# honglianghe/CDNet

Hardware: AMD Instinct MI355X
Metric: tiles/sec (train fwd+bwd+Adam), 256x256 (higher is better)
Workload: dtype fp32

## Files before the change

cdnet_amd/_lib.py:

```python
import ctypes as C
import os

_HERE = os.path.dirname(os.path.abspath(__file__))
LIB_PATH = os.environ.get('CDNET_LIB_PATH') or os.path.join(_HERE, 'libcdnet_hip.so')

_vp, _i, _sz, _f, _u = C.c_void_p, C.c_int, C.c_size_t, C.c_float, C.c_uint

class WgradReduceDesc(C.Structure):
    _fields_ = [('slab', C.c_void_p), ('dw', C.c_void_p)] + [(n, C.c_int) for n in (
        'ksplit', 'npar', 'ci_blocks', 'co_blocks', 'taps', 'CI', 'CO', 'Csrc_real', 'Cin_real', 'src_coff', 'Cout', 'mode', 'block0', 'blocks')]


SIGNATURES = {
    'cdnet_abi_version': (_i, []),
    'cdnet_abi_sizeof': (_sz, [C.c_char_p]),
    'cdnet_last_error': (C.c_char_p, []),
    'cdnet_build_info': (C.c_char_p, []),
    'cdnet_spin': (_i, [_i, _vp]),
    'cdnet_box_copy': (_i, [_vp, _vp, _sz, _vp]),
    'cdnet_box_mfma': (_i, [_vp, _vp, _vp, _i, _i, _i, _vp]),
    'cdnet_ddm_codes': (_i, [_vp, _i, _i, _i, _i, _vp, _i, _i, _vp, _vp, _vp]),
    'cdnet_ddm_normalize': (_i, [_vp, _vp, _i, _i, _i, _vp, _vp]),
    'cdnet_probmaps': (_i, [_vp, _vp, _i, _i, _i, _i, _vp, _vp, _vp]),
    'cdnet_tta_boost_argmax': (_i, [_vp, _vp, _vp, _vp, _i, _i, _vp, _i, _i, _vp, _vp, _vp, _vp, _vp, _vp]),
    'cdnet_fuse_sum': (_i, [_vp, _i, _i, _i, _i, _i, _i, _vp, _i, _i, _vp]),
    'cdnet_upsample_bilinear_backward': (_i, [_vp, _i, _i, _i, _i, _i, _i, _i, _i, _vp, _vp]),
    'cdnet_s2d_to_nhwc': (_i, [_vp, _i, _i, _i, _i, _vp, _vp]),
    'cdnet_fuse_sum_f32': (_i, [_vp, _i, _i, _i, _i, _i, _i, _vp, _i, _i, _vp]),
    'cdnet_upsample_bilinear_backward_f32': (_i, [_vp, _i, _i, _i, _i, _i, _i, _i, _i, _vp, _vp]),
    'cdnet_s2d_to_nhwc_f32': (_i, [_vp, _i, _i, _i, _i, _vp, _vp]),
    'cdnet_bn_backward_stats': (_i, [_vp, _vp, _vp, _vp, _vp, _sz, _vp, _vp]),
    'cdnet_bn_backward_apply': (_i, [_vp, _vp, _vp, _vp]),
    'cdnet_bn_backward_finalize': (_i, [_vp, _vp, _vp, _vp, _vp, _i, _vp, _vp]),
    'cdnet_conv_ws_eligible': (_i, [_vp]),
    'cdnet_grad_sum': (_i, [_vp, _i, _vp, C.c_longlong, _i, _vp, _vp]),
    'cdnet_grad_sum_f32': (_i, [_vp, _i, _vp, C.c_longlong, _i, _vp, _vp]),
    'cdnet_label_pair_histogram': (_i, [_vp, _vp, _i, _i, _i, _i, _vp, _vp, _vp, _vp, _vp, _vp]),
    'cdnet_remap_label': (_i, [_vp, _i, _i, _i, _vp, _vp, _vp, _vp]),
    'cdnet_label_areas': (_i, [_vp, _i, _i, _i, _vp, _vp, _vp]),
    'cdnet_label_apply': (_i, [_vp, _i, _i, _i, _vp, _vp, _vp]),
    'cdnet_label_csr_workspace_bytes': (_sz, [_i]),
    'cdnet_label_csr': (_i, [_vp, _i, _i, _i, _vp, _sz, _vp, _vp, _vp, _vp, _vp]),
    'cdnet_hausdorff_tile_pixels': (_i, []),
    'cdnet_hausdorff_chunk_pixels': (_i, []),
    'cdnet_hausdorff_pairs': (_i, [_vp] * 8 + [_i, _i, _i, _vp, _i, _vp, _i, _vp, _vp, _vp]),
    'cdnet_watershed_workspace_bytes': (_sz, [_i, _i, _i]),
    'cdnet_watershed_process': (_i, [_vp, _i, _i, _i, _i, _vp, _sz, _vp, _vp, _vp, _vp]),
    'cdnet_fill_label_process': (_i, [_vp, _i, _i, _i, _i, _vp, _sz, _vp, _vp]),
    'cdnet_tile_postproc_workspace_bytes': (_sz, [_i, _i, _i, _i]),
    'cdnet_tile_postproc': (_i, [_vp, _vp, _vp, _i, _i, _i, _i, _vp, _i, _i, _i, _i, _vp, _sz] + [_vp] * 10),
    'cdnet_cc_workspace_bytes': (_sz, [_i, _i, _i]),
    'cdnet_cc_chain': (_i, [_vp, _i, _i, _i, _i, _i, _i, _vp, _sz, _vp, _vp, _vp, _vp, _vp, _vp]),
    'cdnet_mask_views_argmax': (_i, [_vp, _i, _i, _i, _vp, _i, _i, _vp, _vp, _vp]),
    'cdnet_tile_mask_postproc_workspace_bytes': (_sz, [_i, _i, _i, _i]),
    'cdnet_tile_mask_postproc': (_i, [_vp, _i, _i, _i, _i, _i, _i, _vp, _sz] + [_vp] * 8),
    'cdnet_dilate_labels': (_i, [_vp, _i, _i, _i, _i, _vp, _vp]),
    'cdnet_conv_packed_weight_elems': (_sz, [_i] * 6),
# ... 122 lines not shown
```

cdnet_amd/csrc/build.py:

```python
import os
import subprocess
import sys

HERE = os.path.dirname(os.path.abspath(__file__))
PKG = os.path.dirname(HERE)
LIB = os.path.join(PKG, 'libcdnet_hip.so')
OBJ_DIR = os.path.join(HERE, 'build')
SOURCES = ['abi.hip', 'box.hip', 'postproc.hip', 'postproc_tile.hip', 'conv.hip', 'conv32.hip', 'conv32ws.hip', 'conv16ws.hip', 'wgrad.hip', 'model.hip', 'head_bwd.hip', 'dam_loss.hip', 'bn_bwd.hip', 'cdm.hip', 'metrics.hip', 'augment.hip', 'optim.hip', 'variance.hip', 'boundary.hip', 'mask_loss.hip']
FLAGS = ['--offload-arch=gfx950', '-O3', '-std=c++20', '-fPIC', '-ffp-contract=off', '-Wall',
         '-Wno-unused-function', '-Wno-unused-result']


def _newer(a, bs):
    return os.path.exists(a) and all(os.path.getmtime(a) >= os.path.getmtime(b) for b in bs)


def build(force=False, verbose=False):
    hipcc = os.environ.get('HIPCC', 'hipcc')
    flags = FLAGS + os.environ.get('CDNET_HIPCC_FLAGS', '').split()
    os.makedirs(OBJ_DIR, exist_ok=True)
    headers = [os.path.join(HERE, f) for f in os.listdir(HERE) if f.endswith('.h')]
    headers.append(os.path.join(os.path.dirname(PKG), 'include', 'cdnet_hip.h'))
    objs, procs = [], []
    for s in SOURCES:
        src = os.path.join(HERE, s)
        if not os.path.exists(src):
            continue
        obj = os.path.join(OBJ_DIR, s.replace('.hip', '.o'))
        objs.append(obj)
        if force or not _newer(obj, [src] + headers):
            cmd = [hipcc] + flags + ['-c', src, '-o', obj]
# ... 17 lines not shown
```

cdnet_amd/csrc/conv32.hip:

```cpp
#include <type_traits>
#include "common.h"
#include "conv_args.h"
#include "launch.h"
#include <stdlib.h>

using namespace cdnet;

typedef __attribute__((ext_vector_type(8))) __bf16 bf16x8;
typedef __attribute__((ext_vector_type(2))) __bf16 bf16x2;
typedef __attribute__((ext_vector_type(16))) float f32x16;
typedef __attribute__((ext_vector_type(2))) float f32x2;
typedef unsigned u32x4 __attribute__((ext_vector_type(4)));
typedef float f32x4 __attribute__((ext_vector_type(4)));

namespace {

__device__ __forceinline__ void split8(const float *v, u32x4 &hi, u32x4 &lo) {
#pragma unroll
    for (int k = 0; k < 4; ++k) {
        const f32x2 x = {v[2 * k], v[2 * k + 1]};
        const bf16x2 h = __builtin_convertvector(x, bf16x2);
        const unsigned hb = __builtin_bit_cast(unsigned, h);
        const f32x2 hf = {__builtin_bit_cast(float, hb << 16), __builtin_bit_cast(float, hb & 0xffff0000u)};
        const bf16x2 l = __builtin_convertvector(x - hf, bf16x2);
// ... 610 lines not shown
                }
#pragma unroll
                for (int q = 0; q < 4; ++q) {
                    const float4 t = xf(raw[q], nullptr);
                    if (q == 0) val = t;
                    else if (ok[q]) { val.x = fmaxf(val.x, t.x); val.y = fmaxf(val.y, t.y); val.z = fmaxf(val.z, t.z); val.w = fmaxf(val.w, t.w); }
                }
            }
        }
        *reinterpret_cast<float4 *>(out + pix * s.C + c) = val;
    }
}

}

namespace cdnet {

int conv_forward_f32(const ConvArgs &A, hipStream_t st) {
    CDNET_REQUIRE(A.CK == 16, "cdnet_conv_forward(f32): CK must be 16 (got %d)", A.CK);
    for (int i = 0; i < A.nsrc; ++i)
        CDNET_REQUIRE(!A.src[i].pool, "cdnet_conv_forward(f32): pooled sources must be materialised (cdnet_src_materialize)");
    CDNET_REQUIRE(!A.out_f16, "cdnet_conv_forward(f32): out_f16 must be 0");
    {
        const int rc = conv_forward_f32_ws(A, st);
        if (rc >= 0) return rc;
    }
    CDNET_REQUIRE(A.ws != 2, "cdnet_conv_forward(f32): the BatchNorm-backward statistics epilogue (ws = 2) needs the producer / consumer kernel "
                             "(ask cdnet_conv_ws_eligible first)");
    CDNET_REQUIRE(A.taps1 == 0 || A.taps1 == A.taps, "cdnet_conv_forward(f32): a one-tap second source runs on conv_ws32_kernel only (ask cdnet_conv_ws_eligible)");
    CDNET_REQUIRE(!A.pool_out, "cdnet_conv_forward(f32): the fused max-pool output rides in conv_ws32_kernel's epilogue only (ask cdnet_conv_ws_eligible)");
    if (A.taps == 9) return dispatch_conv32<9>(A, st);
    if (A.taps == 4) return dispatch_conv32<4>(A, st);
    {
        const int rc = try_conv1x1_stream(A, st);
        if (rc >= 0) return rc;
    }
    return dispatch_conv32<1>(A, st);
}

int materialize_f32(const ConvSrc &s, int N, int H, int W, void *out, hipStream_t st) {
    const size_t total = (size_t)N * H * W * (s.C / 4);
    size_t g = (total + 255) / 256;
    g = g > 8192 ? 8192 : g;
    materialize_f32_kernel<<<(int)g, 256, 0, st>>>(s, N, H, W, reinterpret_cast<float *>(out));
    return check_launch("cdnet_src_materialize(f32)");
}

// ... 2 lines not shown
```

cdnet_amd/csrc/conv_args.h:

```cpp
#pragma once
#include "../../include/cdnet_hip.h"

struct ConvSrc {
    const unsigned short *x;
    const unsigned short *res;
    const float *scale;
    const float *shift;
    int C, Hs, Ws, pool, relu, off_y, off_x;
    int f16, row_stride;
};

struct ConvArgs {
    ConvSrc src[2];
    int nsrc;
    const unsigned short *w;
    const float *bias;
    const float *oscale;
    const float *oshift;
    int orelu;
    unsigned short *out;
    int Cout, out_cstride, out_coff;
    float *stats;
    int N, H, W;
    int taps, npar, ostride, nchunk;
    int tile, CK, BN;
    int out_f16;
    int debug;
    int ws;
    int f32;
    const unsigned short *eres;
    const float *eres_scale, *eres_shift;
    int eres_f16, eres_relu;
    int taps1, pad_;
    unsigned short *pool_out;
    const float *dot_w, *dot_b;
    float *dot_out;
};

enum : int {
    CONV_DBG_WS16_QUAD = 16,
    CONV_DBG_ONE_TILE = 32,
    CONV_DBG_PERSIST_SMALL = 64,
    CONV_DBG_OLD_WS16 = 128,
    CONV_DBG_NO_STREAM_1X1 = 256,
    CONV_DBG_GRID_SHIFT = 8,
};
enum : int {
    WGRAD_DBG_NO_WS = 8,
    WGRAD_DBG_ALL_QUADS = 16,
};

static_assert(sizeof(ConvSrc) == sizeof(cdnet_conv_src), "ConvSrc layout");
static_assert(sizeof(ConvArgs) == sizeof(cdnet_conv_args), "ConvArgs layout");

namespace cdnet {
int conv_forward_f32(const ConvArgs &A, hipStream_t st);
int conv_forward_f32_ws(const ConvArgs &A, hipStream_t st, bool dry_run = false);
int conv_forward_ws16(const ConvArgs &A, hipStream_t st, bool dry_run = false);
int materialize_f32(const ConvSrc &s, int N, int H, int W, void *out, hipStream_t st);
}
```

cdnet_amd/engine.py:

```python
import ctypes as C
import os
import torch

from . import _lib


class ConvSrc(C.Structure):
    _fields_ = [('x', C.c_void_p), ('res', C.c_void_p), ('scale', C.c_void_p), ('shift', C.c_void_p),
                ('C', C.c_int), ('Hs', C.c_int), ('Ws', C.c_int), ('pool', C.c_int), ('relu', C.c_int),
                ('off_y', C.c_int), ('off_x', C.c_int), ('f16', C.c_int), ('row_stride', C.c_int)]


class ConvArgs(C.Structure):
    _fields_ = [('src', ConvSrc * 2), ('nsrc', C.c_int), ('w', C.c_void_p), ('bias', C.c_void_p),
                ('oscale', C.c_void_p), ('oshift', C.c_void_p), ('orelu', C.c_int), ('out', C.c_void_p),
                ('Cout', C.c_int), ('out_cstride', C.c_int), ('out_coff', C.c_int), ('stats', C.c_void_p),
                ('N', C.c_int), ('H', C.c_int), ('W', C.c_int), ('taps', C.c_int), ('npar', C.c_int),
                ('ostride', C.c_int), ('nchunk', C.c_int), ('tile', C.c_int), ('CK', C.c_int), ('BN', C.c_int),
                ('out_f16', C.c_int), ('debug', C.c_int), ('ws', C.c_int), ('f32', C.c_int),
                ('eres', C.c_void_p), ('eres_scale', C.c_void_p), ('eres_shift', C.c_void_p), ('eres_f16', C.c_int), ('eres_relu', C.c_int),
                ('taps1', C.c_int), ('pad_', C.c_int), ('pool_out', C.c_void_p),
                ('dot_w', C.c_void_p), ('dot_b', C.c_void_p), ('dot_out', C.c_void_p)]


def _dp(t):
    return None if t is None else t.data_ptr()


class Src:

    def __init__(self, x, scale=None, shift=None, relu=False, pool=False, res=None, off=(0, 0), view=None):
        assert x.dtype in (torch.bfloat16, torch.float16, torch.float32) and x.is_contiguous()
        assert res is None or res.dtype == x.dtype
        self.x, self.scale, self.shift, self.relu, self.pool, self.res, self.off = x, scale, shift, relu, pool, res, off
        if view is None:
            assert x.dim() == 4
            self.N, self.Hs, self.Ws, self.Cc = x.shape
            self.ptr_off, self.row_stride = 0, 0
        else:
            self.ptr_off, self.Hs, self.Ws, self.Cc, self.row_stride = view
            self.N = x.shape[0]

    @property
    def f16(self):
# ... 125 lines not shown
            wp = torch.zeros((Cout, Cin_p, KH, KW), dtype=torch.float32, device=w.device)
            wp[:, :Cin] = w
        else:
            raise NotImplementedError
        w, Cin = wp.contiguous(), Cin_p
    n = packed_elems(Cout, Cin // CK, taps, CK, BN, npar) * (2 if split else 1)
    if out is None or out.numel() != n:
        out = torch.empty((n,), dtype=torch.int16, device=w.device)
    if cout_scale is not None:
        assert mode == 0 and cout_scale.dtype == torch.float32 and cout_scale.numel() == Cout
        _lib.call('cdnet_pack_conv_weights_scaled', _lib.ptr(w), _lib.ptr(cout_scale), _lib.ptr(out), Cout, Cin, KH, KW, CK, BN,
                  mode | (PACK_SPLIT if split else 0), _lib.stream_ptr())
        return out
    _lib.call('cdnet_pack_conv_weights', _lib.ptr(w), _lib.ptr(out), Cout, Cin, KH, KW, CK, BN, mode | (PACK_SPLIT if split else 0),
              _lib.stream_ptr())
    return out


CONV_DEBUG = 0


def conv_forward(srcs, wpacked, Cout, cfg, taps=9, transposed=False, bias=None, oscale=None, oshift=None,
                 orelu=False, out=None, stats=None, H=None, W=None, out_dtype=torch.bfloat16, eres=None, query_ws=False, bns=None, taps1=0, pool_out=None, dot=None,
                 pad_chunks=0, debug_or=0):
    tile, CK, BN = cfg[:3]
    s0 = srcs[0]
    f32 = s0.f32
    assert all(s.f32 == f32 for s in srcs)
    if f32:
        out_dtype = torch.float32
    N = s0.N
    if H is None:
        H, W = s0.logical_hw()
        H, W = H + 0, W + 0
    ostride = 2 if transposed else 1
    npar = 4 if transposed else 1
    a = ConvArgs()
    nchunk = 0
    for i, s in enumerate(srcs):
        assert s.C % CK == 0, (s.C, CK)
        s.fill(a.src[i])
        nchunk += s.C // CK
    a.nsrc = len(srcs)
    if dot is not None:
        assert out is None and stats is None and eres is None and bns is None and pool_out is None and not f32 and not transposed
        a.dot_w, a.dot_b, a.dot_out = dot[0].data_ptr(), dot[1].data_ptr(), dot[2].data_ptr()
        assert dot[0].numel() == Cout and dot[0].dtype == torch.float32 and dot[2].dtype == torch.float32 and dot[2].numel() == N * H * W
    elif out is None:
        out = torch.empty((N, H * ostride, W * ostride, Cout), dtype=out_dtype, device=s0.x.device)
    ntiles = ((H + tile - 1) // tile) * ((W + tile - 1) // tile)
    if stats is True:
        stats = torch.empty((N * npar * ntiles, 2, Cout), dtype=torch.float32, device=s0.x.device)
    a.w, a.bias, a.oscale, a.oshift = _dp(wpacked), _dp(bias), _dp(oscale), _dp(oshift)
    a.orelu = int(orelu)
    a.out, a.Cout, a.out_cstride, a.out_coff = (None if out is None else out.data_ptr()), Cout, (Cout if out is None else out.shape[3]), 0
    a.stats = _dp(stats)
    a.N, a.H, a.W = N, H, W
    assert pad_chunks == 0 or (len(srcs) == 2 and taps == 9 and not f32 and all(s.scale is None and not s.relu and s.res is None and not s.f16 for s in srcs))
    a.taps, a.npar, a.ostride, a.nchunk = taps, npar, ostride, nchunk + pad_chunks
    a.tile, a.CK, a.BN = tile, CK, BN
    a.out_f16 = int(out is not None and out.dtype == torch.float16)
    a.ws = 0
    a.taps1 = taps1
    a.pool_out = _dp(pool_out)
    a.debug = CONV_DEBUG | debug_or
    a.f32 = int(f32)
    assert out is None or (out.dtype == torch.float32) == f32
    if eres is not None:
        assert not transposed and stats is None and not orelu and out.dtype == (torch.float32 if f32 else torch.bfloat16) and tuple(eres.x.shape) == tuple(out.shape)
        assert eres.f32 == f32
        a.eres, a.eres_scale, a.eres_shift = eres.x.data_ptr(), _dp(eres.scale), _dp(eres.shift)
        a.eres_f16, a.eres_relu = int(eres.f16), int(eres.relu)
    if bns is not None:
        raw, sc, sh, mu, inv, partial = bns
        assert eres is None and stats is None and bias is None and oscale is None and oshift is None and tuple(raw.shape) == tuple(out.shape)
        a.ws = 2
        a.eres, a.oscale, a.oshift, a.eres_scale, a.eres_shift, a.stats = raw.data_ptr(), sc.data_ptr(), sh.data_ptr(), mu.data_ptr(), inv.data_ptr(), partial.data_ptr()
    if query_ws:
        return int(_lib.load().cdnet_conv_ws_eligible(C.byref(a)))
    _lib.call('cdnet_conv_forward', C.byref(a), _lib.stream_ptr())
    return out, stats
```

cdnet_amd/trainer.py:

```python
import ctypes as C
import os

import torch

from . import _lib, engine, optim, runtime, streams
from .allreduce import BucketReducer, bucketed_allreduce
from .engine import Src
from .optim import HEAD_PARAMS, FlatState
from .synth import synthetic_batch


class GradIn(C.Structure):
    _fields_ = [('g', C.c_void_p), ('Hg', C.c_int), ('Wg', C.c_int), ('oy', C.c_int), ('ox', C.c_int),
                ('pooled', C.c_int), ('coff', C.c_int), ('cstride', C.c_int), ('pad_', C.c_int)]


class BnBwdArgs(C.Structure):
    _fields_ = [('raw', C.c_void_p), ('res', C.c_void_p), ('scale', C.c_void_p), ('shift', C.c_void_p),
                ('mean', C.c_void_p), ('invstd', C.c_void_p), ('gin', GradIn * 3), ('ngin', C.c_int),
                ('f16', C.c_int), ('relu', C.c_int), ('N', C.c_int), ('H', C.c_int), ('W', C.c_int), ('C', C.c_int)]


_WGRAD_WGS_DEEP, _WGRAD_WGS_SHALLOW = 128, 160
_WGRAD_WGS_KQ = 128
# ... 575 lines not shown
        wpb, cfgb = L.backward_pack(cin_total, H, W)
        if L.kind == 'conv3s2':
            Cp = cin_total // 4
            gs2d = self.buf(('ds2d', L.name), (N, H, W, cin_total), runtime.act_dtype())
            engine.conv_forward([Src(g)], wpb, cin_total, cfgb, taps=9, out=gs2d, H=H, W=W)
            gin = self.buf(('din', L.name), (N, 2 * H, 2 * W, Cp), runtime.act_dtype())
            _lib.call(_lib.entry('cdnet_s2d_to_nhwc', gin.dtype == torch.float32), _lib.ptr(gs2d), N, H, W, Cp, _lib.ptr(gin),
                      _lib.stream_ptr())
            add(srcs[0].x, _G(gin, 2 * H, 2 * W))
            return
        if not L.transposed:
            gin = self.buf(('din', L.name), (N, H, W, cin_total), runtime.act_dtype())
            fuse = None if isinstance(g, Src) else self._stats_fusable(L, srcs, H, W, N, wpb, cfgb, cin_total)
            if fuse is not None:
                P, part = fuse
                engine.conv_forward([Src(g)], wpb, cin_total, cfgb, taps=L.taps, out=gin, H=H, W=W,
                                    bns=(srcs[0].x, P.scale, P.shift, P.save_mean, P.save_invstd, part))
                self._bn_partials[id(srcs[0].x)] = part
            else:
                engine.conv_forward([g if isinstance(g, Src) else Src(g)], wpb, cin_total, cfgb, taps=L.taps, out=gin, H=H, W=W)
        else:
            gin = self.buf(('din', L.name), (N, H, W, cin_total), runtime.act_dtype())
            views = [Src(g, view=(a * 2 * W * Cout, H, W, 2 * Cout, 4 * W * Cout)) for a in (0, 1)]
            engine.conv_forward(views, wpb, cin_total, cfgb, taps=(9 if L.kind == 'convT4' else 1), out=gin, H=H, W=W)
        coff = 0
        for s in srcs:
            if getattr(s, 'is_input', False):
                coff += s.C
                continue
            tgt, pool = getattr(s, 'grad_to', (s.x, int(s.pool)))
            add(tgt, _G(gin, H, W, oy=s.off[0], ox=s.off[1], pooled=pool, coff=coff, cstride=cin_total))
            coff += s.C

    def _overlap_begin(self):
        self._ar = None
        if not self._reduce_active() or os.environ.get('CDNET_ALLREDUCE_OVERLAP', '1') == '0':
            return
        f = self.flat
        base = f.G.data_ptr()
        pend = {}
        owners = [p for L in self.tape if not isinstance(L, runtime.FuseNode) for p in (L.weight, L.bias, None if L.bn is None else L.bn.weight,
                                                 None if L.bn is None else L.bn.bias) if p is not None]
        for p in owners:
            off = (p.grad.data_ptr() - base) // 4
            if 0 <= off < f.n_used:
                pend[off] = off + p.numel()
        if f.n_head:
# ... 204 lines not shown
```

include/cdnet_hip.h:

```cpp
#ifndef CDNET_HIP_H
#define CDNET_HIP_H

#include <stddef.h>
#include <stdint.h>

#ifdef __cplusplus
extern "C" {
#endif

#define CDNET_OK            0
#define CDNET_E_ARG         1
#define CDNET_E_WORKSPACE   2
#define CDNET_E_LAUNCH      3

#define CDNET_ABI_VERSION   5

int         cdnet_abi_version(void);
size_t      cdnet_abi_sizeof(const char *struct_name);
const char *cdnet_last_error(void);
const char *cdnet_build_info(void);
int         cdnet_spin(int microseconds, void *stream);
int         cdnet_box_copy(const void *src, void *dst, size_t bytes, void *stream);
int         cdnet_box_mfma(const uint32_t *seed, float *sink, unsigned long long *stamps, int workgroups, int waves_per_wg, int iters, void *stream);

// ... 56 lines not shown
    int nsrc;
    const uint16_t *w;
    const float *bias;
    const float *oscale;
    const float *oshift;
    int orelu;
    uint16_t *out;
    int Cout, out_cstride, out_coff;
    float *stats;
    int N, H, W;
    int taps;
    int npar;
    int ostride;
    int nchunk;
    int tile, CK, BN;
    int out_f16;
    int debug;
    int ws;
    int f32;
    const uint16_t *eres;
    const float *eres_scale, *eres_shift;
    int eres_f16, eres_relu;
    int taps1;
    int pad_;
    uint16_t *pool_out;
    const float *dot_w;
    const float *dot_b;
    float *dot_out;
} cdnet_conv_args;

size_t cdnet_conv_packed_weight_elems(int Cout, int nchunk, int taps, int CK, int BN, int npar);
#define CDNET_PACK_SPLIT 16
int cdnet_pack_conv_weights(const float *w, void *packed, int Cout, int Cin, int KH, int KW, int CK, int BN, int mode,
                            void *stream);
int cdnet_pack_conv_weights_scaled(const float *w, const float *cout_scale, void *packed, int Cout, int Cin, int KH, int KW, int CK,
                                   int BN, int mode, void *stream);
typedef struct cdnet_pack_job {
    const float *w;
    void *packed;
    int Cout, Cin, KH, KW, CK, BN, mode, pad_;
} cdnet_pack_job;
size_t cdnet_pack_batch_table_bytes(int n_jobs);
int cdnet_pack_conv_weights_batch(const cdnet_pack_job *jobs, int n_jobs, void *table, size_t table_bytes, int upload,
                                  void *stream);
int cdnet_conv_forward(const cdnet_conv_args *args, void *stream);

int cdnet_input_pack(const float *x, int N, int C, int H, int W, void *out_bf16_nhwc16, void *stream);
// ... 8 lines not shown
typedef struct cdnet_head_feat {
    const uint16_t *raw;
    const uint16_t *res;
    const float *scale;
    const float *shift;
    int relu;
    int f16;
} cdnet_head_feat;

#define CDNET_HEAD_WEIGHT_FLOATS 855
int cdnet_dam_head_forward(const cdnet_head_feat *f1, const cdnet_head_feat *f2, const cdnet_head_feat *f3,
                           const float *head_weights, int N, int H, int W, float *mask, float *point,
                           float *direction, void *stream);
int cdnet_final_conv1x1(const cdnet_head_feat *f, const float *w, const float *b, int K, int N, int H, int W,
                        float *out, void *stream);
size_t cdnet_bias_grad_workspace_floats(int C);
int cdnet_bias_grad(const uint16_t *grad_out, size_t npix, int C, float *workspace, size_t workspace_floats, float *db, void *stream);
int cdnet_bias_grad_f32(const float *grad_out, size_t npix, int C, float *workspace, size_t workspace_floats, float *db, void *stream);
size_t cdnet_final_conv1x1_backward_workspace_floats(void);
int cdnet_final_conv1x1_backward(const cdnet_head_feat *f, const float *w, const float *dlogits, int K, int N, int H, int W,
                                 uint16_t *df, float *workspace, size_t workspace_floats, float *dw, float *db, void *stream);

int cdnet_conv_ws_eligible(const cdnet_conv_args *args);

int cdnet_src_materialize(const cdnet_conv_src *src, int N, int H, int W, uint16_t *out, void *stream);

size_t cdnet_conv_wgrad_slab_floats(int C_src, int Cout, int taps, int npar, int ci_tiles, int ksplit);
int cdnet_conv_backward_weight(const cdnet_conv_src *src, int src_coff, int Csrc_real, int Cin_real,
                               const uint16_t *grad_out, int Cout, int N, int H, int W, int taps, int npar,
                               int ostride, int ci_tiles, int ksplit, float *slab, float *dw, int mode, void *stream);

#define CDNET_WGRAD_DEFER_REDUCE 0x100
typedef struct cdnet_wgrad_reduce_desc {
    const float *slab;
    float *dw;
    int ksplit, npar, ci_blocks, co_blocks, taps, CI, CO, Csrc_real, Cin_real, src_coff, Cout, mode;
    int block0, blocks;
} cdnet_wgrad_reduce_desc;
int cdnet_wgrad_reduce_desc_fill(int C_src, int src_coff, int Csrc_real, int Cin_real, int Cout, int taps, int npar, int ci_tiles,
                                 int ksplit, const float *slab, float *dw, int mode, int block0, cdnet_wgrad_reduce_desc *out);
int cdnet_wgrad_reduce_batch(const cdnet_wgrad_reduce_desc *table_dev, int n, int total_blocks, void *stream);

typedef struct cdnet_grad_in {
    const uint16_t *g;
    int Hg, Wg;
    int oy, ox;
// ... 185 lines not shown
```

Baseline: 1068.

## Add dedicated fp32 transposed-conv kernels exploiting stride-2 tap sparsity

Adds a new convt32 source holding specialised MFMA kernels for the 2x2 transposed conv (4 taps, 4 parities). The forward kernel writes all four output parities from a single halo tile. The backward-data kernel computes only the 4 non-zero taps per channel chunk instead of a dense 9-tap conv. The aim is to skip the zero-weight taps and redundant work that the generic conv path spends on these layers. Costs are a new code path with its own correctness risks. CONV_DBG_NO_CONVT4 is given the same bit value as CONV_DBG_OLD_WS16 (128), so a debug flag now toggles two behaviours.

```diff
diff --git a/cdnet_amd/_lib.py b/cdnet_amd/_lib.py
--- a/cdnet_amd/_lib.py
+++ b/cdnet_amd/_lib.py
@@ -33,6 +33,8 @@
     'cdnet_bn_backward_apply': (_i, [_vp, _vp, _vp, _vp]),
     'cdnet_bn_backward_finalize': (_i, [_vp, _vp, _vp, _vp, _vp, _i, _vp, _vp]),
     'cdnet_conv_ws_eligible': (_i, [_vp]),
+    'cdnet_convt32_launches': (C.c_longlong, [_i]),
+    'cdnet_convt32_scratch_bytes': (_i, []),
     'cdnet_grad_sum': (_i, [_vp, _i, _vp, C.c_longlong, _i, _vp, _vp]),
     'cdnet_grad_sum_f32': (_i, [_vp, _i, _vp, C.c_longlong, _i, _vp, _vp]),
     'cdnet_label_pair_histogram': (_i, [_vp, _vp, _i, _i, _i, _i, _vp, _vp, _vp, _vp, _vp, _vp]),
diff --git a/cdnet_amd/csrc/build.py b/cdnet_amd/csrc/build.py
--- a/cdnet_amd/csrc/build.py
+++ b/cdnet_amd/csrc/build.py
@@ -6,7 +6,7 @@
 PKG = os.path.dirname(HERE)
 LIB = os.path.join(PKG, 'libcdnet_hip.so')
 OBJ_DIR = os.path.join(HERE, 'build')
-SOURCES = ['abi.hip', 'box.hip', 'postproc.hip', 'postproc_tile.hip', 'conv.hip', 'conv32.hip', 'conv32ws.hip', 'conv16ws.hip', 'wgrad.hip', 'model.hip', 'head_bwd.hip', 'dam_loss.hip', 'bn_bwd.hip', 'cdm.hip', 'metrics.hip', 'augment.hip', 'optim.hip', 'variance.hip', 'boundary.hip', 'mask_loss.hip']
+SOURCES = ['abi.hip', 'box.hip', 'postproc.hip', 'postproc_tile.hip', 'conv.hip', 'conv32.hip', 'convt32.hip', 'conv32ws.hip', 'conv16ws.hip', 'wgrad.hip', 'model.hip', 'head_bwd.hip', 'dam_loss.hip', 'bn_bwd.hip', 'cdm.hip', 'metrics.hip', 'augment.hip', 'optim.hip', 'variance.hip', 'boundary.hip', 'mask_loss.hip']
 FLAGS = ['--offload-arch=gfx950', '-O3', '-std=c++20', '-fPIC', '-ffp-contract=off', '-Wall',
          '-Wno-unused-function', '-Wno-unused-result']
 
diff --git a/cdnet_amd/csrc/conv32.hip b/cdnet_amd/csrc/conv32.hip
--- a/cdnet_amd/csrc/conv32.hip
+++ b/cdnet_amd/csrc/conv32.hip
@@ -656,7 +656,15 @@
         CDNET_REQUIRE(!A.src[i].pool, "cdnet_conv_forward(f32): pooled sources must be materialised (cdnet_src_materialize)");
     CDNET_REQUIRE(!A.out_f16, "cdnet_conv_forward(f32): out_f16 must be 0");
     {
+        const int rc = try_convt4_fwd(A, st);
+        if (rc >= 0) return rc;
+    }
+    {
         const int rc = conv_forward_f32_ws(A, st);
+        if (rc >= 0) return rc;
+    }
+    {
+        const int rc = try_convt4_bwd(A, st);
         if (rc >= 0) return rc;
     }
     CDNET_REQUIRE(A.ws != 2, "cdnet_conv_forward(f32): the BatchNorm-backward statistics epilogue (ws = 2) needs the producer / consumer kernel "
diff --git a/cdnet_amd/csrc/conv_args.h b/cdnet_amd/csrc/conv_args.h
--- a/cdnet_amd/csrc/conv_args.h
+++ b/cdnet_amd/csrc/conv_args.h
@@ -31,7 +31,7 @@
     const unsigned short *eres;
     const float *eres_scale, *eres_shift;
     int eres_f16, eres_relu;
-    int taps1, pad_;
+    int taps1, convt_bwd;
     unsigned short *pool_out;
     const float *dot_w, *dot_b;
     float *dot_out;
@@ -42,6 +42,7 @@
     CONV_DBG_ONE_TILE = 32,
     CONV_DBG_PERSIST_SMALL = 64,
     CONV_DBG_OLD_WS16 = 128,
+    CONV_DBG_NO_CONVT4 = 128,
     CONV_DBG_NO_STREAM_1X1 = 256,
     CONV_DBG_GRID_SHIFT = 8,
 };
@@ -58,4 +59,6 @@
 int conv_forward_f32_ws(const ConvArgs &A, hipStream_t st, bool dry_run = false);
 int conv_forward_ws16(const ConvArgs &A, hipStream_t st, bool dry_run = false);
 int materialize_f32(const ConvSrc &s, int N, int H, int W, void *out, hipStream_t st);
+int try_convt4_fwd(const ConvArgs &A, hipStream_t st);
+int try_convt4_bwd(const ConvArgs &A, hipStream_t st);
 }
diff --git a/cdnet_amd/csrc/convt32.hip b/cdnet_amd/csrc/convt32.hip
--- /dev/null
+++ b/cdnet_amd/csrc/convt32.hip
@@ -0,0 +1,589 @@
+#include <type_traits>
+#include "common.h"
+#include "conv_args.h"
+#include "launch.h"
+
+using namespace cdnet;
+
+typedef __attribute__((ext_vector_type(8))) __bf16 bf16x8;
+typedef __attribute__((ext_vector_type(2))) __bf16 bf16x2;
+typedef __attribute__((ext_vector_type(16))) float f32x16;
+typedef __attribute__((ext_vector_type(2))) float f32x2;
+typedef unsigned u32x4 __attribute__((ext_vector_type(4)));
+typedef float f32x4 __attribute__((ext_vector_type(4)));
+
+namespace {
+
+long long g_launches[2];
+
+__device__ __forceinline__ void split8(const float *v, u32x4 &hi, u32x4 &lo) {
+#pragma unroll
+    for (int k = 0; k < 4; ++k) {
+        const f32x2 x = {v[2 * k], v[2 * k + 1]};
+        const bf16x2 h = __builtin_convertvector(x, bf16x2);
+        const unsigned hb = __builtin_bit_cast(unsigned, h);
+        const f32x2 hf = {__builtin_bit_cast(float, hb << 16), __builtin_bit_cast(float, hb & 0xffff0000u)};
+        const bf16x2 l = __builtin_convertvector(x - hf, bf16x2);
+        hi[k] = hb;
+        lo[k] = __builtin_bit_cast(unsigned, l);
+    }
+}
+
+constexpr int CK = 16;
+constexpr int PSTR = CK * 2 + 16;
+constexpr int XF_MAX = 2048;
+
+template <int TH, int TW>
+struct Halo {
+    static constexpr int HW_ = TW + 2, NPIX = (TH + 2) * (TW + 2);
+    static constexpr int VPP = CK / 8;
+    static constexpr int NA = (NPIX * VPP + 255) / 256;
+    static constexpr int A_PLANE = NPIX * PSTR;
+};
+
+template <int TH, int TW>
+__device__ __forceinline__ void halo_geometry(const ConvArgs &A, int y0, int x0, int tid, int (&eoff)[Halo<TH, TW>::NA]) {
+    using G = Halo<TH, TW>;
+    const int slot = tid % G::VPP;
+    const ConvSrc &s = A.src[0];
+    const int rs = s.row_stride ? s.row_stride : s.Ws * s.C;
+#pragma unroll
+    for (int i = 0; i < G::NA; ++i) {
+        const int v = tid + i * 256;
+        const int pix = v / G::VPP;
+        const int hy = pix / G::HW_, hx = pix - hy * G::HW_;
+        const int y = y0 - 1 + hy, x = x0 - 1 + hx;
+        const int ys = y - s.off_y, xs = x - s.off_x;
+        const bool ok = v < G::NPIX * G::VPP && (unsigned)y < (unsigned)A.H && (unsigned)x < (unsigned)A.W && (unsigned)ys < (unsigned)s.Hs &&
+                        (unsigned)xs < (unsigned)s.Ws;
+        eoff[i] = ok ? ys * rs + xs * s.C + slot * 8 : -1;
+    }
+}
+
+template <int TH, int TW>
+__device__ __forceinline__ void halo_request(const ConvSrc &s, int n, int cc0, const int (&eoff)[Halo<TH, TW>::NA],
+                                             f32x4 (&pa)[Halo<TH, TW>::NA][2]) {
+    const size_t rs = s.row_stride ? (size_t)s.row_stride : (size_t)s.Ws * s.C;
+    const float *base = reinterpret_cast<const float *>(s.x) + (size_t)n * s.Hs * rs + cc0;
+#pragma unroll
+    for (int i = 0; i < Halo<TH, TW>::NA; ++i) {
+        const int e = eoff[i];
+        const f32x4 *p = reinterpret_cast<const f32x4 *>(base + (e >= 0 ? e : 0));
+        pa[i][0] = p[0];
+        pa[i][1] = p[1];
+    }
+}
+
+template <int TH, int TW>
+__device__ __forceinline__ void halo_commit(const ConvSrc &s, int n, int cc0, const float *xf, int xfs, const int (&eoff)[Halo<TH, TW>::NA],
+                                            const f32x4 (&pa)[Halo<TH, TW>::NA][2], unsigned char *lds_a, int tid) {
+    using G = Halo<TH, TW>;
+    constexpr int NA = G::NA, VPP = G::VPP;
+    const int slot = tid % VPP;
+    const bool on = s.scale != nullptr, relu = s.relu != 0;
+    float sc[8], sh[8];
+    if (on) {
+#pragma unroll
+        for (int j = 0; j < 8; ++j) { sc[j] = xf[j]; sh[j] = xf[xfs + j]; }
+    }
+    f32x4 rr[NA][2];
+    if (s.res) {
+        const size_t rs = s.row_stride ? (size_t)s.row_stride : (size_t)s.Ws * s.C;
+        const float *rbase = reinterpret_cast<const float *>(s.res) + (size_t)n * s.Hs * rs + cc0;
+#pragma unroll
+        for (int i = 0; i < NA; ++i) {
+            const int e = eoff[i];
+            const f32x4 *p = reinterpret_cast<const f32x4 *>(rbase + (e >= 0 ? e : 0));
+            rr[i][0] = p[0];
+            rr[i][1] = p[1];
+        }
+    }
+    unsigned char *dst0 = lds_a + (tid / VPP) * PSTR + slot * 16;
+#pragma unroll
+    for (int i = 0; i < NA; ++i) {
+        if (tid + i * 256 >= G::NPIX * VPP) continue;
+        const int e = eoff[i];
+        u32x4 hi = {0u, 0u, 0u, 0u}, lo = {0u, 0u, 0u, 0u};
+        if (e >= 0) {
+            float v[8] = {pa[i][0][0], pa[i][0][1], pa[i][0][2], pa[i][0][3], pa[i][1][0], pa[i][1][1], pa[i][1][2], pa[i][1][3]};
+            if (on) {
+#pragma unroll
+                for (int j = 0; j < 8; ++j) v[j] = fmaf(v[j], sc[j], sh[j]);
+            }
+            if (s.res) {
+                const float r[8] = {rr[i][0][0], rr[i][0][1], rr[i][0][2], rr[i][0][3], rr[i][1][0], rr[i][1][1], rr[i][1][2], rr[i][1][3]};
+#pragma unroll
+                for (int j = 0; j < 8; ++j) v[j] += r[j];
+            }
+            if (relu) {
+#pragma unroll
+                for (int j = 0; j < 8; ++j) v[j] = fmaxf(v[j], 0.f);
+            }
+            split8(v, hi, lo);
+        }
+        unsigned char *d = dst0 + i * (256 / VPP) * PSTR;
+        *reinterpret_cast<u32x4 *>(d) = hi;
+        *reinterpret_cast<u32x4 *>(d + G::A_PLANE) = lo;
+    }
+}
+
+__device__ __forceinline__ void fill_xf(const ConvArgs &A, float *s_xf, int c0n, int ctot, int xfs, int tid) {
+    for (int c = tid; c < ctot; c += 256) {
+        const ConvSrc &S = c < c0n ? A.src[0] : A.src[1];
+        const int cc = c < c0n ? c : c - c0n;
+        s_xf[c] = S.scale ? S.scale[cc] : 1.f;
+        s_xf[xfs + c] = S.shift ? S.shift[cc] : 0.f;
+    }
+}
+
+__device__ __forceinline__ void xcd_order(int &tile, int &cout_tile) {
+    const int NC = (int)gridDim.y, lin = (int)blockIdx.y * (int)gridDim.x + (int)blockIdx.x;
+    const int T = (int)gridDim.x * NC, q = T >> 3, rem = T & 7;
+    const int xcd = lin & 7, idx = lin >> 3;
+    const int seq = xcd < rem ? xcd * (q + 1) + idx : rem * (q + 1) + (xcd - rem) * q + idx;
+    tile = seq / NC;
+    cout_tile = seq - tile * NC;
+}
+
+template <int TH, int TW, int BN>
+struct LdsBwd {
+    static constexpr int TB = CK * BN * 2;
+    static constexpr int B_PLANE = 4 * TB;
+    static constexpr int MAIN = (2 * Halo<TH, TW>::A_PLANE + 2 * B_PLANE + 15) / 16 * 16;
+    static int bytes(int ctot) { return MAIN + 2 * ((ctot + 7) / 8 * 8) * 4; }
+};
+
+template <int MPW, int NPW, int TW>
+__device__ __forceinline__ void store_tile(const ConvArgs &A, const f32x16 (&acc)[MPW][NPW], int n, int y0, int x0, int mblock0, int nblock0,
+                                           int half, int l31, int cout0) {
+    float *out = reinterpret_cast<float *>(A.out);
+    const bool full = y0 + 16 <= A.H && x0 + TW <= A.W && cout0 + (nblock0 + NPW) * 32 <= A.Cout && TW == 16;
+    if (full) {
+        const int cs = A.out_cstride;
+        float *tb = out + (((size_t)n * A.H + y0) * A.W + x0) * cs + A.out_coff;
+#pragma unroll
+        for (int ni = 0; ni < NPW; ++ni) {
+            const int co = cout0 + (nblock0 + ni) * 32 + l31;
+            const float osc = A.oscale ? A.oscale[co] : 1.f;
+            const float osh = fmaf(A.bias ? A.bias[co] : 0.f, osc, A.oshift ? A.oshift[co] : 0.f);
+            float *ob = tb + co;
+#pragma unroll
+            for (int mi = 0; mi < MPW; ++mi) {
+                const int rowb = ((mblock0 + mi) * 2) * A.W + 4 * half;
+#pragma unroll
+                for (int r = 0; r < 16; ++r) {
+                    const int p = (r & 3) + 8 * (r >> 2);
+                    const int off = (rowb + (p / 16) * A.W + (p % 16)) * cs;
+                    float v = fmaf(acc[mi][ni][r], osc, osh);
+                    if (A.orelu) v = fmaxf(v, 0.f);
+                    ob[off] = v;
+                }
+            }
+        }
+        return;
+    }
+#pragma unroll
+    for (int ni = 0; ni < NPW; ++ni) {
+        const int co = cout0 + (nblock0 + ni) * 32 + l31;
+        const bool cok = co < A.Cout;
+        const float osc = (A.oscale && cok) ? A.oscale[co] : 1.f;
+        const float osh = fmaf((A.bias && cok) ? A.bias[co] : 0.f, osc, (A.oshift && cok) ? A.oshift[co] : 0.f);
+#pragma unroll
+        for (int mi = 0; mi < MPW; ++mi) {
+#pragma unroll
+            for (int r = 0; r < 16; ++r) {
+                const int m = (mblock0 + mi) * 32 + (r & 3) + 8 * (r >> 2) + 4 * half;
+                const int y = y0 + m / TW, x = x0 + m % TW;
+                float v = fmaf(acc[mi][ni][r], osc, osh);
+                if (A.orelu) v = fmaxf(v, 0.f);
+                if (cok && y < A.H && x < A.W) out[(((size_t)n * A.H + y) * A.W + x) * A.out_cstride + A.out_coff + co] = v;
+            }
+        }
+    }
+}
+
+template <int TH, int TW, int BN, int WM, int WN>
+__global__ __launch_bounds__(256, 2) void convt4_f32_bwd_kernel(ConvArgs A) {
+    using G = Halo<TH, TW>;
+    using L = LdsBwd<TH, TW, BN>;
+    constexpr int HW_ = G::HW_, NA = G::NA;
+    constexpr int MT = TH * TW / 32, NT = BN / 32;
+    constexpr int MPW = MT / WM, NPW = NT / WN;
+    constexpr int TBV = L::TB / 16;
+    constexpr int NBV = 2 * 4 * TBV;
+    constexpr int NB = (NBV + 255) / 256;
+    constexpr int B_PACK = 9 * L::TB;
+    static_assert(MT % WM == 0 && NT % WN == 0 && WM * WN == 4, "wave tiling");
+
+    extern __shared__ __attribute__((aligned(16))) unsigned char smem[];
+    unsigned char *lds_a = smem;
+    unsigned char *lds_b = smem + 2 * G::A_PLANE;
+    float *s_xf = reinterpret_cast<float *>(smem + L::MAIN);
+
+    const int tid = threadIdx.x, lane = tid & 63, wave = tid >> 6;
+    const int wm = wave / WN, wn = wave % WN;
+    const int half = lane >> 5, l31 = lane & 31;
+    const int c0n = A.src[0].C, ctot = 2 * c0n;
+    const int xfs = (ctot + 7) / 8 * 8;
+    fill_xf(A, s_xf, c0n, ctot, xfs, tid);
+
+    const int tiles_x = (A.W + TW - 1) / TW, tiles_y = (A.H + TH - 1) / TH;
+    const int tiles_img = tiles_x * tiles_y;
+    int tile, cout_tile;
+    xcd_order(tile, cout_tile);
+    const int n = tile / tiles_img, rt = tile - n * tiles_img;
+    const int ty_ = rt / tiles_x;
+    const int y0 = ty_ * TH, x0 = (rt - ty_ * tiles_x) * TW;
+
+    int eoff[NA];
+    halo_geometry<TH, TW>(A, y0, x0, tid, eoff);
+    const int n0 = c0n / CK, nb = n0 / 2;
+    const unsigned short *wbase = A.w + ((size_t)cout_tile * A.nchunk) * (size_t)B_PACK;
+
+    f32x4 pa[NA][2];
+    u32x4 pb[NB];
+    auto issue = [&](int chunk) {
+        const int si = chunk >= n0, cl = chunk - si * n0, b = cl >= nb;
+        halo_request<TH, TW>(A.src[si], n, cl * CK, eoff, pa);
+        const u32x4 *wsrc = reinterpret_cast<const u32x4 *>(wbase + (size_t)chunk * B_PACK);
+        const int tap0 = (1 - si) * 3 + (1 - b);
+#pragma unroll
+        for (int i = 0; i < NB; ++i) {
+            const int v = tid + i * 256;
+            const int hl = v / (4 * TBV), t = (v / TBV) & 3, wi = v % TBV;
+            const int tap = tap0 + (t >> 1) * 3 + (t & 1);
+            if (v < NBV) pb[i] = wsrc[hl * (B_PACK / 16) + tap * TBV + wi];
+        }
+    };
+    auto commit = [&](int chunk) {
+        const int si = chunk >= n0, cc0 = (chunk - si * n0) * CK;
+        halo_commit<TH, TW>(A.src[si], n, cc0, s_xf + (si ? c0n : 0) + cc0 + (tid % G::VPP) * 8, xfs, eoff, pa, lds_a, tid);
+        u32x4 *bdst = reinterpret_cast<u32x4 *>(lds_b);
+#pragma unroll
+        for (int i = 0; i < NB; ++i) {
+            const int v = tid + i * 256;
+            if (v < NBV) bdst[v] = pb[i];
+        }
+    };
+
+    int abase[MPW];
+#pragma unroll
+    for (int mi = 0; mi < MPW; ++mi) {
+        const int m = (wm * MPW + mi) * 32 + l31;
+        abase[mi] = ((m / TW) * HW_ + m % TW) * PSTR + half * 16;
+    }
+    const int bbase = half * BN * 16 + (wn * NPW * 32 + l31) * 16;
+    f32x16 acc[MPW][NPW];
+#pragma unroll
+    for (int mi = 0; mi < MPW; ++mi)
+#pragma unroll
+        for (int ni = 0; ni < NPW; ++ni)
+#pragma unroll
+            for (int r = 0; r < 16; ++r) acc[mi][ni][r] = 0.f;
+
+    issue(0);
+    for (int chunk = 0; chunk < A.nchunk; ++chunk) {
+        __syncthreads();
+        commit(chunk);
+        __syncthreads();
+        if (chunk + 1 < A.nchunk) issue(chunk + 1);
+        const int si = chunk >= n0, b = (chunk - si * n0) >= nb;
+        const unsigned char *pa0 = lds_a + ((1 - si) * HW_ + (1 - b)) * PSTR;
+#pragma unroll
+        for (int t = 0; t < 4; ++t) {
+            const int toff = ((t >> 1) * HW_ + (t & 1)) * PSTR;
+            bf16x8 ah[MPW], al[MPW], bh[NPW], bl[NPW];
+#pragma unroll
+            for (int mi = 0; mi < MPW; ++mi) {
+                ah[mi] = *reinterpret_cast<const bf16x8 *>(pa0 + abase[mi] + toff);
+                al[mi] = *reinterpret_cast<const bf16x8 *>(pa0 + G::A_PLANE + abase[mi] + toff);
+            }
+#pragma unroll
+            for (int ni = 0; ni < NPW; ++ni) {
+                bh[ni] = *reinterpret_cast<const bf16x8 *>(lds_b + bbase + t * L::TB + ni * 512);
+                bl[ni] = *reinterpret_cast<const bf16x8 *>(lds_b + L::B_PLANE + bbase + t * L::TB + ni * 512);
+            }
+#pragma unroll
+            for (int mi = 0; mi < MPW; ++mi)
+#pragma unroll
+                for (int ni = 0; ni < NPW; ++ni) {
+                    acc[mi][ni] = __builtin_amdgcn_mfma_f32_32x32x16_bf16(al[mi], bh[ni], acc[mi][ni], 0, 0, 0);
+                    acc[mi][ni] = __builtin_amdgcn_mfma_f32_32x32x16_bf16(ah[mi], bl[ni], acc[mi][ni], 0, 0, 0);
+                    acc[mi][ni] = __builtin_amdgcn_mfma_f32_32x32x16_bf16(ah[mi], bh[ni], acc[mi][ni], 0, 0, 0);
+                }
+        }
+    }
+    store_tile<MPW, NPW, TW>(A, acc, n, y0, x0, wm * MPW, wn * NPW, half, l31, cout_tile * BN);
+}
+
+template <int TH, int TW, int BN, int WM, int WN>
+int launch_convt4_bwd(const ConvArgs &A, hipStream_t st) {
+    using L = LdsBwd<TH, TW, BN>;
+    dim3 grid(cdiv(A.W, TW) * cdiv(A.H, TH) * A.N, cdiv(A.Cout, BN), 1);
+    const int rc = launch_lds<convt4_f32_bwd_kernel<TH, TW, BN, WM, WN>>(grid, 256, L::bytes(XF_MAX), L::bytes(2 * A.src[0].C), st,
+                                                                         "hipFuncSetAttribute(convt4_bwd)", "convt4_f32_bwd_kernel", A);
+    if (rc == CDNET_OK) ++g_launches[1];
+    return rc;
+}
+
+template <int TH, int TW, int BN>
+struct LdsFwd {
+    static constexpr int TB = CK * BN * 2;
+    static constexpr int B_PAR = 2 * 4 * TB;
+    static constexpr int STAGE = 2 * Halo<TH, TW>::A_PLANE + 4 * B_PAR;
+    static constexpr int STATS_BYTES = 4 * 4 * 2 * BN * 4;
+    static constexpr int MAIN = ((STAGE > STATS_BYTES ? STAGE : STATS_BYTES) + 15) / 16 * 16;
+    static int bytes(int ctot) { return MAIN + 2 * ((ctot + 7) / 8 * 8) * 4; }
+};
+
+template <int TH, int TW, int BN, int WM, int WN>
+__global__ __launch_bounds__(256, 2) void convt4_f32_fwd_kernel(ConvArgs A, int bnp) {
+    using G = Halo<TH, TW>;
+    using L = LdsFwd<TH, TW, BN>;
+    constexpr int HW_ = G::HW_, NA = G::NA;
+    constexpr int MT = TH * TW / 32, NT = BN / 32;
+    constexpr int MPW = MT / WM, NPW = NT / WN;
+    constexpr int TBV = L::TB / 16;
+    constexpr int NBV = 4 * 2 * 4 * TBV;
+    constexpr int NB = NBV / 256;
+    static_assert(MT % WM == 0 && NT % WN == 0 && WM * WN == 4 && NBV % 256 == 0, "wave tiling");
+
+    extern __shared__ __attribute__((aligned(16))) unsigned char smem[];
+    unsigned char *lds_a = smem;
+    unsigned char *lds_b = smem + 2 * G::A_PLANE;
+    float (*s_stats)[4][2][BN] = reinterpret_cast<float (*)[4][2][BN]>(smem);
+    float *s_xf = reinterpret_cast<float *>(smem + L::MAIN);
+
+    const int tid = threadIdx.x, lane = tid & 63, wave = tid >> 6;
+    const int wm = wave / WN, wn = wave % WN;
+    const int half = lane >> 5, l31 = lane & 31;
+    const ConvSrc &S = A.src[0];
+    const int ctot = S.C;
+    const int xfs = (ctot + 7) / 8 * 8;
+    fill_xf(A, s_xf, ctot, ctot, xfs, tid);
+
+    const int tiles_x = (A.W + TW - 1) / TW, tiles_y = (A.H + TH - 1) / TH;
+    const int tiles_img = tiles_x * tiles_y;
+    int tile, cout_tile;
+    xcd_order(tile, cout_tile);
+    const int n = tile / tiles_img, rt = tile - n * tiles_img;
+    const int ty_ = rt / tiles_x;
+    const int y0 = ty_ * TH, x0 = (rt - ty_ * tiles_x) * TW;
+
+    int eoff[NA];
+    halo_geometry<TH, TW>(A, y0, x0, tid, eoff);
+
+    const int cout0 = cout_tile * BN;
+    const int ptile = cout0 / bnp, pcol0 = cout0 - ptile * bnp, ptiles = (A.Cout + bnp - 1) / bnp;
+    const size_t par_stride = (size_t)ptiles * A.nchunk * (size_t)(CK * bnp);
+    const u32x4 *wbase = reinterpret_cast<const u32x4 *>(A.w) + (size_t)ptile * A.nchunk * (size_t)(CK * bnp);
+    constexpr int VPAR = 2 * 4 * TBV;
+    static_assert(256 % TBV == 0 || TBV % 256 == 0, "a thread's vectors differ by whole images");
+    const int woff0 = (((tid / TBV) & 7) * 2 + ((tid / BN) & 1)) * bnp + pcol0 + tid % BN;
+
+    f32x4 pa[NA][2];
+    u32x4 pb[NB];
+    auto issue = [&](int chunk) {
+        halo_request<TH, TW>(S, n, chunk * CK, eoff, pa);
+        const u32x4 *wsrc = wbase + (size_t)chunk * (CK * bnp);
+#pragma unroll
+        for (int i = 0; i < NB; ++i)
+            pb[i] = wsrc[(i * 256 / VPAR) * par_stride + woff0 + ((i * 256 / TBV) & 7) * 2 * bnp];
+    };
+    auto commit = [&](int chunk) {
+        const int cc0 = chunk * CK;
+        halo_commit<TH, TW>(S, n, cc0, s_xf + cc0 + (tid % G::VPP) * 8, xfs, eoff, pa, lds_a, tid);
+        u32x4 *bdst = reinterpret_cast<u32x4 *>(lds_b);
+#pragma unroll
+        for (int i = 0; i < NB; ++i) bdst[tid + i * 256] = pb[i];
+    };
+
+    int abase[MPW];
+#pragma unroll
+    for (int mi = 0; mi < MPW; ++mi) {
+        const int m = (wm * MPW + mi) * 32 + l31;
+        abase[mi] = ((m / TW) * HW_ + m % TW) * PSTR + half * 16;
+    }
+    const int bbase = half * BN * 16 + (wn * NPW * 32 + l31) * 16;
+    f32x16 acc[4][MPW][NPW];
+#pragma unroll
+    for (int p = 0; p < 4; ++p)
+#pragma unroll
+        for (int mi = 0; mi < MPW; ++mi)
+#pragma unroll
+            for (int ni = 0; ni < NPW; ++ni)
+#pragma unroll
+                for (int r = 0; r < 16; ++r) acc[p][mi][ni][r] = 0.f;
+
+    issue(0);
+    for (int chunk = 0; chunk < A.nchunk; ++chunk) {
+        __syncthreads();
+        commit(chunk);
+        __syncthreads();
+        if (chunk + 1 < A.nchunk) issue(chunk + 1);
+#pragma unroll
+        for (int pos = 8; pos >= 0; --pos) {
+            const int r = pos / 3, c = pos % 3;
+            bf16x8 ah[MPW], al[MPW];
+#pragma unroll
+            for (int mi = 0; mi < MPW; ++mi) {
+                ah[mi] = *reinterpret_cast<const bf16x8 *>(lds_a + abase[mi] + (r * HW_ + c) * PSTR);
+                al[mi] = *reinterpret_cast<const bf16x8 *>(lds_a + G::A_PLANE + abase[mi] + (r * HW_ + c) * PSTR);
+            }
+#pragma unroll
+            for (int p = 0; p < 4; ++p) {
+                const int a = p >> 1, b = p & 1;
+                const int ty = (a ? 2 : 1) - r, tx = (b ? 2 : 1) - c;
+                if (ty < 0 || ty > 1 || tx < 0 || tx > 1) continue;
+                const int t = ty * 2 + tx;
+                bf16x8 bh[NPW], bl[NPW];
+#pragma unroll
+                for (int ni = 0; ni < NPW; ++ni) {
+                    bh[ni] = *reinterpret_cast<const bf16x8 *>(lds_b + p * L::B_PAR + bbase + t * L::TB + ni * 512);
+                    bl[ni] = *reinterpret_cast<const bf16x8 *>(lds_b + p * L::B_PAR + 4 * L::TB + bbase + t * L::TB + ni * 512);
+                }
+#pragma unroll
+                for (int mi = 0; mi < MPW; ++mi)
+#pragma unroll
+                    for (int ni = 0; ni < NPW; ++ni) {
+                        acc[p][mi][ni] = __builtin_amdgcn_mfma_f32_32x32x16_bf16(al[mi], bh[ni], acc[p][mi][ni], 0, 0, 0);
+                        acc[p][mi][ni] = __builtin_amdgcn_mfma_f32_32x32x16_bf16(ah[mi], bl[ni], acc[p][mi][ni], 0, 0, 0);
+                        acc[p][mi][ni] = __builtin_amdgcn_mfma_f32_32x32x16_bf16(ah[mi], bh[ni], acc[p][mi][ni], 0, 0, 0);
+                    }
+            }
+        }
+    }
+    __syncthreads();
+
+    if (A.stats) {
+#pragma unroll
+        for (int p = 0; p < 4; ++p)
+#pragma unroll
+            for (int ni = 0; ni < NPW; ++ni) {
+                float ssum = 0.f, ssq = 0.f;
+#pragma unroll
+                for (int mi = 0; mi < MPW; ++mi)
+#pragma unroll
+                    for (int r = 0; r < 16; ++r) {
+                        const int m = (wm * MPW + mi) * 32 + (r & 3) + 8 * (r >> 2) + 4 * half;
+                        const float v = ((y0 + m / TW) < A.H && (x0 + m % TW) < A.W) ? acc[p][mi][ni][r] : 0.f;
+                        ssum += v;
+                        ssq = fmaf(v, v, ssq);
+                    }
+                ssum += __shfl_xor(ssum, 32);
+                ssq += __shfl_xor(ssq, 32);
+                if (half == 0) {
+                    s_stats[p][wave][0][(wn * NPW + ni) * 32 + l31] = ssum;
+                    s_stats[p][wave][1][(wn * NPW + ni) * 32 + l31] = ssq;
+                }
+            }
+        __syncthreads();
+        for (int i = tid; i < 4 * 2 * BN; i += 256) {
+            const int p = i / (2 * BN), which = (i / BN) & 1, col = i % BN;
+            const int wn_of = col / (NPW * 32);
+            float v = 0.f;
+#pragma unroll
+            for (int k = 0; k < WM; ++k) v += s_stats[p][k * WN + wn_of][which][col];
+            const int co = cout0 + col;
+            const size_t row = (size_t)(n * 4 + p) * tiles_img + rt;
+            if (co < A.Cout) A.stats[(row * 2 + which) * A.Cout + co] = v;
+        }
+    }
+    float *out = reinterpret_cast<float *>(A.out);
+    const int Wo = 2 * A.W;
+#pragma unroll
+    for (int ni = 0; ni < NPW; ++ni) {
+        const int co = cout0 + (wn * NPW + ni) * 32 + l31;
+        const bool cok = co < A.Cout;
+        const float osc = (A.oscale && cok) ? A.oscale[co] : 1.f;
+        const float osh = fmaf((A.bias && cok) ? A.bias[co] : 0.f, osc, (A.oshift && cok) ? A.oshift[co] : 0.f);
+        float *oc = out + A.out_coff + co;
+#pragma unroll
+        for (int mi = 0; mi < MPW; ++mi) {
+#pragma unroll
+            for (int r = 0; r < 16; ++r) {
+                const int m = (wm * MPW + mi) * 32 + (r & 3) + 8 * (r >> 2) + 4 * half;
+                const int y = y0 + m / TW, x = x0 + m % TW;
+                const bool ok = cok && y < A.H && x < A.W;
+                float *op = oc + (((size_t)n * 2 * A.H + 2 * y) * Wo + 2 * x) * A.out_cstride;
+#pragma unroll
+                for (int p = 0; p < 4; ++p) {
+                    float v = fmaf(acc[p][mi][ni][r], osc, osh);
+                    if (A.orelu) v = fmaxf(v, 0.f);
+                    if (ok) op[((size_t)(p >> 1) * Wo + (p & 1)) * A.out_cstride] = v;
+                }
+            }
+        }
+    }
+}
+
+template <int TH, int TW, int BN, int WM, int WN>
+int launch_convt4_fwd(const ConvArgs &A, hipStream_t st) {
+    using L = LdsFwd<TH, TW, BN>;
+    dim3 grid(cdiv(A.W, TW) * cdiv(A.H, TH) * A.N, cdiv(A.Cout, BN), 1);
+    const int rc = launch_lds<convt4_f32_fwd_kernel<TH, TW, BN, WM, WN>>(grid, 256, L::bytes(XF_MAX), L::bytes(A.src[0].C), st,
+                                                                         "hipFuncSetAttribute(convt4_fwd)", "convt4_f32_fwd_kernel", A, A.BN);
+    if (rc == CDNET_OK) ++g_launches[0];
+    return rc;
+}
+
+bool plain_size(const ConvArgs &A) {
+    long long ctot = 0;
+    for (int i = 0; i < A.nsrc; ++i) {
+        const ConvSrc &s = A.src[i];
+        const long long rs = s.row_stride ? s.row_stride : (long long)s.Ws * s.C;
+        if ((long long)s.Hs * rs >= (1LL << 31)) return false;
+        ctot += s.C;
+    }
+    return ctot <= XF_MAX;
+}
+
+}
+
+namespace cdnet {
+
+int try_convt4_fwd(const ConvArgs &A, hipStream_t st) {
+    if (A.debug & CONV_DBG_NO_CONVT4) return -1;
+    if (!A.f32 || A.taps != 4 || A.taps1 != 0 || A.npar != 4 || A.ostride != 2 || A.nsrc != 1 || A.ws || A.eres || A.pool_out || A.dot_out) return -1;
+    if (A.CK != CK || A.src[0].pool || A.src[0].C != A.nchunk * CK || !plain_size(A)) return -1;
+    if (A.tile != 16 || (A.BN != 64 && A.BN != 32)) return -1;
+    if (!(A.debug & CONV_DBG_PERSIST_SMALL)) {
+        int n_cu = 0;
+        if (const int rc = cu_count(&n_cu)) return rc;
+        if ((long long)cdiv(A.W, 16) * cdiv(A.H, 16) * A.N * cdiv(A.Cout, 32) < n_cu) return -1;
+    }
+    return launch_convt4_fwd<16, 16, 32, 4, 1>(A, st);
+}
+
+int try_convt4_bwd(const ConvArgs &A, hipStream_t st) {
+    if (A.debug & CONV_DBG_NO_CONVT4) return -1;
+    if (!A.f32 || A.convt_bwd != 1 || A.taps != 9 || A.taps1 != 0 || A.npar != 1 || A.ostride != 1 || A.nsrc != 2 || A.ws || A.stats || A.eres ||
+        A.pool_out || A.dot_out)
+        return -1;
+    const int c = A.src[0].C;
+    const ConvSrc &s0 = A.src[0], &s1 = A.src[1];
+    if (s0.Hs != s1.Hs || s0.Ws != s1.Ws || s0.off_y != s1.off_y || s0.off_x != s1.off_x || s0.row_stride != s1.row_stride) return -1;
+    if (A.CK != CK || A.src[1].C != c || c % (2 * CK) != 0 || A.nchunk * CK != 2 * c || A.src[0].pool || A.src[1].pool || !plain_size(A)) return -1;
+    if (A.tile == 16 && A.BN == 64) return launch_convt4_bwd<16, 16, 64, 4, 1>(A, st);
+    if (A.tile == 16 && A.BN == 32) return launch_convt4_bwd<16, 16, 32, 4, 1>(A, st);
+    if (A.tile == 8 && A.BN == 64) return launch_convt4_bwd<8, 8, 64, 2, 2>(A, st);
+    return -1;
+}
+
+}
+
+extern "C" long long cdnet_convt32_launches(int part) {
+    return (part == 0 || part == 1) ? g_launches[part] : -1;
+}
+
+extern "C" int cdnet_convt32_scratch_bytes(void) {
+    const void *kernels[] = {reinterpret_cast<const void *>(convt4_f32_fwd_kernel<16, 16, 32, 4, 1>), reinterpret_cast<const void *>(convt4_f32_bwd_kernel<16, 16, 64, 4, 1>),
+                             reinterpret_cast<const void *>(convt4_f32_bwd_kernel<16, 16, 32, 4, 1>), reinterpret_cast<const void *>(convt4_f32_bwd_kernel<8, 8, 64, 2, 2>)};
+    int most = 0;
+    for (const void *k : kernels) {
+        hipFuncAttributes at;
+        if (hipFuncGetAttributes(&at, k) != hipSuccess) return -1;
+        most = (int)at.localSizeBytes > most ? (int)at.localSizeBytes : most;
+    }
+    return most;
+}
diff --git a/cdnet_amd/engine.py b/cdnet_amd/engine.py
--- a/cdnet_amd/engine.py
+++ b/cdnet_amd/engine.py
@@ -19,7 +19,7 @@
                 ('ostride', C.c_int), ('nchunk', C.c_int), ('tile', C.c_int), ('CK', C.c_int), ('BN', C.c_int),
                 ('out_f16', C.c_int), ('debug', C.c_int), ('ws', C.c_int), ('f32', C.c_int),
                 ('eres', C.c_void_p), ('eres_scale', C.c_void_p), ('eres_shift', C.c_void_p), ('eres_f16', C.c_int), ('eres_relu', C.c_int),
-                ('taps1', C.c_int), ('pad_', C.c_int), ('pool_out', C.c_void_p),
+                ('taps1', C.c_int), ('convt_bwd', C.c_int), ('pool_out', C.c_void_p),
                 ('dot_w', C.c_void_p), ('dot_b', C.c_void_p), ('dot_out', C.c_void_p)]
 
 
@@ -191,7 +191,7 @@
 
 def conv_forward(srcs, wpacked, Cout, cfg, taps=9, transposed=False, bias=None, oscale=None, oshift=None,
                  orelu=False, out=None, stats=None, H=None, W=None, out_dtype=torch.bfloat16, eres=None, query_ws=False, bns=None, taps1=0, pool_out=None, dot=None,
-                 pad_chunks=0, debug_or=0):
+                 pad_chunks=0, debug_or=0, convt_bwd=False):
     tile, CK, BN = cfg[:3]
     s0 = srcs[0]
     f32 = s0.f32
@@ -231,6 +231,8 @@
     a.out_f16 = int(out is not None and out.dtype == torch.float16)
     a.ws = 0
     a.taps1 = taps1
+    assert not convt_bwd or (taps == 9 and len(srcs) == 2 and not transposed)
+    a.convt_bwd = int(convt_bwd)
     a.pool_out = _dp(pool_out)
     a.debug = CONV_DEBUG | debug_or
     a.f32 = int(f32)
diff --git a/cdnet_amd/trainer.py b/cdnet_amd/trainer.py
--- a/cdnet_amd/trainer.py
+++ b/cdnet_amd/trainer.py
@@ -621,7 +621,8 @@
         else:
             gin = self.buf(('din', L.name), (N, H, W, cin_total), runtime.act_dtype())
             views = [Src(g, view=(a * 2 * W * Cout, H, W, 2 * Cout, 4 * W * Cout)) for a in (0, 1)]
-            engine.conv_forward(views, wpb, cin_total, cfgb, taps=(9 if L.kind == 'convT4' else 1), out=gin, H=H, W=W)
+            engine.conv_forward(views, wpb, cin_total, cfgb, taps=(9 if L.kind == 'convT4' else 1), out=gin, H=H, W=W,
+                                convt_bwd=(L.kind == 'convT4'))
         coff = 0
         for s in srcs:
             if getattr(s, 'is_input', False):
diff --git a/include/cdnet_hip.h b/include/cdnet_hip.h
--- a/include/cdnet_hip.h
+++ b/include/cdnet_hip.h
@@ -102,7 +102,7 @@
     const float *eres_scale, *eres_shift;
     int eres_f16, eres_relu;
     int taps1;
-    int pad_;
+    int convt_bwd;
     uint16_t *pool_out;
     const float *dot_w;
     const float *dot_b;
@@ -157,6 +157,8 @@
                                  uint16_t *df, float *workspace, size_t workspace_floats, float *dw, float *db, void *stream);
 
 int cdnet_conv_ws_eligible(const cdnet_conv_args *args);
+long long cdnet_convt32_launches(int part);
+int cdnet_convt32_scratch_bytes(void);
 
 int cdnet_src_materialize(const cdnet_conv_src *src, int N, int H, int W, uint16_t *out, void *stream);
 
```

New measurement: 1074, median of 6. About the same (+0.6%).
